# AjayGaneshC/medical-segmentation-pytorch

Hardware: AMD Instinct MI355X
Metric: images/sec (whole node) + val Dice, DUCKNet-17 352x352 at 1/2/4/8 MI355X (higher is better)
Workload: dtype bf16; 1 GPU; model=DUCKNet-17, global_batch=320, per_gpu_batch=320, seq_len=123904, step=SegTrainer.train_step, image_size=352, parallelism=dp1, impl=fused, optimizer=adam, loss=ce, syncbn=False, hipgraph=True

## Files before the change

csrc/bindings.cpp:

```cpp
#include <torch/extension.h>
#include <c10/hip/HIPStream.h>

#include <algorithm>
#include <vector>

#include "launchers.h"

namespace {

hipStream_t cur_stream() { return c10::hip::getCurrentHIPStream().stream(); }

#define CHECK_DEV(t) TORCH_CHECK((t).is_cuda() && (t).is_contiguous(), #t " must be a contiguous GPU tensor")
#define CHECK_BF16(t) CHECK_DEV(t); TORCH_CHECK((t).scalar_type() == at::kBFloat16, #t " must be bf16")
#define CHECK_F32(t) CHECK_DEV(t); TORCH_CHECK((t).scalar_type() == at::kFloat, #t " must be fp32")
#define CHECK_I64(t) CHECK_DEV(t); TORCH_CHECK((t).scalar_type() == at::kLong, #t " must be int64")

inline uint16_t* bf(const at::Tensor& t) { return reinterpret_cast<uint16_t*>(t.data_ptr()); }
inline float* f32(const at::Tensor& t) { return t.data_ptr<float>(); }
inline const float* f32_opt(const c10::optional<at::Tensor>& t) {
  if (!t.has_value() || !t->defined()) return nullptr;
  CHECK_F32(*t);
  return t->data_ptr<float>();
}
inline float* f32_opt_mut(const c10::optional<at::Tensor>& t) { return const_cast<float*>(f32_opt(t)); }

using OptTensors = std::vector<c10::optional<at::Tensor>>;

void fill_coefs(const OptTensors& cs, int n, const std::vector<int64_t>& ld, const float** out) {
  TORCH_CHECK(cs.empty() || (int)cs.size() == n, "one prologue entry per input");
  for (int i = 0; i < n; ++i) {
    out[i] = nullptr;
    if (cs.empty() || !cs[i].has_value() || !cs[i]->defined()) continue;
    CHECK_F32(*cs[i]);
    TORCH_CHECK(cs[i]->numel() >= 2 * ld[i], "prologue coefficients must hold [scale; shift] rows of the input width");
    out[i] = cs[i]->data_ptr<float>();
  }
}

bool fill_bwd(const OptTensors& ys, const OptTensors& ss, const OptTensors& ks, int n, int64_t numel, int64_t C,
// ... 1590 lines not shown
PYBIND11_MODULE(_C, m) {
  m.doc() = "MI355X (gfx950) HIP kernels for medical_segmentation_pytorch_amd";
  m.def("conv_fwd", &conv_fwd, py::arg("xs"), py::arg("wp"), py::arg("ys"), py::arg("bias"), py::arg("stat_part"),
        py::arg("dims"), py::arg("dy"), py::arg("dx"), py::arg("trans"), py::arg("xc") = OptTensors{},
        py::arg("xrelu") = 0, py::arg("accumulate") = false, py::arg("gy") = OptTensors{},
        py::arg("gs") = OptTensors{}, py::arg("gk") = OptTensors{}, py::arg("grelu") = 0);
  m.def("conv_fwd_bn", &conv_fwd_bn, py::arg("xs"), py::arg("wp"), py::arg("ys"), py::arg("stat_part"), py::arg("dims"),
        py::arg("dy"), py::arg("dx"), py::arg("bn_y"), py::arg("bn_coef"), py::arg("relu"), py::arg("gy") = OptTensors{},
        py::arg("gs") = OptTensors{}, py::arg("gk") = OptTensors{}, py::arg("grelu") = 0);
  m.def("conv_wgrad", &conv_wgrad_t, py::arg("dys"), py::arg("xs"), py::arg("dw"), py::arg("dims"), py::arg("dy"),
        py::arg("dx"), py::arg("trans"), py::arg("xc") = OptTensors{}, py::arg("xrelu") = 0,
        py::arg("gy") = OptTensors{}, py::arg("gs") = OptTensors{}, py::arg("gk") = OptTensors{}, py::arg("grelu") = 0);
  m.def("conv_wgrad_uses_halo", &conv_wgrad_uses_halo_t);
  m.def("conv_pick_mi", &conv_pick_mi);
  m.def("conv_rows_alloc", &conv_rows_alloc);
  m.def("conv_stat_blocks", &conv_stat_blocks_t, py::arg("dims"), py::arg("dy"), py::arg("dx"), py::arg("trans") = false,
        py::arg("bwd") = false, py::arg("bne") = false);
  m.def("conv_uses_halo", &conv_uses_halo_t, py::arg("dims"), py::arg("dy"), py::arg("dx"), py::arg("trans"),
        py::arg("bwd") = false);
  m.def("conv_set_halo", [](bool on) { conv_set_halo(on ? 1 : 0); });
  m.def("conv_set_halo_split", [](int64_t mode) { conv_set_halo_split((int)mode); });
  m.def("conv_set_gemm", [](bool on) { conv_gemm_set(on ? 1 : 0); });
  m.def("conv_gemm_force_cfg", [](int64_t c) { conv_gemm_force_cfg((int)c); });
  m.def("conv_gemm_num_cfgs", []() { return conv_gemm_num_cfgs(); });
  m.def("conv_gemm_stamp_buffer", [](c10::optional<at::Tensor> buf) {
    if (!buf.has_value()) return conv_gemm_stamp_buffer(nullptr, 0);
    TORCH_CHECK(buf->is_cuda() && buf->is_contiguous() && buf->scalar_type() == at::kLong && buf->dim() == 2 &&
                    buf->size(1) == 4, "conv_gemm_stamp_buffer: a contiguous int64 [blocks][4] device tensor");
    return conv_gemm_stamp_buffer(buf->data_ptr(), buf->size(0));
  });
  m.def("conv_set_wgrad_gemm", [](int64_t mode) { conv_wgrad_gemm_set((int)mode); });
  m.def("conv_wgrad_gemm_force_cfg", [](int64_t c) { conv_wgrad_gemm_force_cfg((int)c); });
  m.def("conv_wgrad_gemm_num_cfgs", []() { return conv_wgrad_gemm_num_cfgs(); });
  m.def("conv_uses_wgrad_gemm", [](std::vector<int64_t> dims, std::vector<int64_t> dy, std::vector<int64_t> dx, bool trans) {
    return conv_wgrad_gemm_ok(make_geom(dims, dy, dx), trans);
  });
  m.def("conv_uses_gemm", [](std::vector<int64_t> dims, std::vector<int64_t> dy, std::vector<int64_t> dx, bool trans) {
    return conv_gemm_ok(make_geom(dims, dy, dx), trans);
  });
  m.def("conv_set_phase", [](bool on) { conv_set_phase(on ? 1 : 0); });
  m.def("pack_weight", &pack_weight_t);
  m.def("unpack_wgrad", &unpack_wgrad_t, py::arg("src"), py::arg("dst"), py::arg("nrow"), py::arg("nch"),
        py::arg("T"), py::arg("Cpk"), py::arg("Ktot"), py::arg("t_base"), py::arg("c_base"), py::arg("s_row"),
        py::arg("s_ch"), py::arg("accumulate"), py::arg("nrep") = 1, py::arg("rep_stride") = 0);
  m.def("conv_wgrad_replicas", &conv_wgrad_replicas_t, py::arg("dims"), py::arg("dy"), py::arg("dx"), py::arg("trans"),
        py::arg("bwd") = false, py::arg("pro") = false);
  m.def("pack_batch", &pack_batch_t);
  m.def("pack_per_block", &pack_per_block);
  m.def("bn_partial_blocks", [](int64_t P, int64_t Cp) { return bn_partial_blocks(P, Cp); });
  m.def("sum_stats", &sum_stats_t, py::arg("inputs"), py::arg("out"), py::arg("part"), py::arg("P"), py::arg("Cp"),
        py::arg("coefs") = OptTensors{}, py::arg("relu_mask") = 0);
  m.def("bn_reduce_partials", &bn_reduce_partials_t);
  m.def("bn_reduce_splits", [](int64_t nblk) { return bn_reduce_splits(nblk); });
  m.def("bn_collapse", &bn_collapse_t);
  m.def("bn_finalize", &bn_finalize_t);
  m.def("bn_reduce_finalize", &bn_reduce_finalize_t);
  m.def("bn_reduce_bwd_finalize", &bn_reduce_bwd_finalize_t);
  m.def("bn_rf_chunks", [](int64_t Cp) { return bn_rf_chunks((int)Cp); });
  m.def("bn_act_apply", &bn_act_apply_t);
  m.def("bn_act_apply_relu6", &bn_act_apply_relu6_t);
  m.def("bn_add_act", &bn_add_act_t);
  m.def("gconv_fwd", &gconv_fwd_t);
  m.def("relu6", &relu6_t);
  m.def("relu6_bwd", &relu6_bwd_t);
  m.def("bn_aug_mask", &bn_aug_mask_t);
  m.def("gconv_dgrad", &gconv_dgrad_t);
// ... 155 lines not shown
```

csrc/build.py:

```python
#!/usr/bin/env python3
from __future__ import annotations

import argparse
import os
import shutil
import subprocess
import sys
import sysconfig

HERE = os.path.dirname(os.path.abspath(__file__))
ROOT = os.path.dirname(HERE)
PKG = os.path.join(ROOT, 'medical_segmentation_pytorch_amd')
VARIANT = os.environ.get('MSP_BUILD_VARIANT', '')
BUILD = os.path.join(ROOT, 'build', 'csrc' + (f'_{VARIANT}' if VARIANT else ''))
ARCH = os.environ.get('PYTORCH_ROCM_ARCH', 'gfx950').split(';')[0]
ROCM = os.environ.get('ROCM_PATH', '/opt/rocm')


def source_files():
    names = sorted(f for f in os.listdir(HERE) if f.endswith(('.hip', '.h', '.cpp')))
    return [os.path.join(HERE, f) for f in names] + [os.path.abspath(__file__)]


def sources_sha():
# ... 39 lines not shown
    tdir = os.path.dirname(torch.__file__)
    inc = [os.path.join(tdir, 'include'), os.path.join(tdir, 'include', 'torch', 'csrc', 'api', 'include')]
    return tdir, inc, int(torch._C._GLIBCXX_USE_CXX11_ABI)


def write_ninja(jobs):
    tdir, tinc, abi = torch_paths()
    pyinc = sysconfig.get_paths()['include']
    import pybind11
    hipcc = shutil.which('hipcc') or os.path.join(ROCM, 'bin', 'hipcc')
    kernels = sorted(f for f in os.listdir(HERE) if f.endswith('.hip'))
    common = f'-O3 -fPIC -std=c++17 -D_GLIBCXX_USE_CXX11_ABI={abi} -I{HERE}'
    kflags = f'{common} --offload-arch={ARCH} -munsafe-fp-atomics -Wno-unused-result'
    if VARIANT:
        kflags += ' ' + os.environ.get('MSP_BUILD_DEFINES', '')
    bflags = (f'{common} -D__HIP_PLATFORM_AMD__=1 -DUSE_ROCM=1 -DTORCH_EXTENSION_NAME=_C '
              f'-DTORCH_API_INCLUDE_EXTENSION_H -I{ROCM}/include -I{pyinc} -I{pybind11.get_include()} '
              + ' '.join(f'-isystem {p}' for p in tinc) + ' -Wno-deprecated-declarations')
    tlib = os.path.join(tdir, 'lib')
    ldflags = (f'-shared -fPIC -L{tlib} -Wl,-rpath,{tlib} -Wl,--no-as-needed -lc10 -ltorch -ltorch_cpu '
               f'-ltorch_python -lc10_hip -ltorch_hip')
    out = os.path.join(PKG, '_C.so') if not VARIANT else os.path.join(ROOT, 'build', VARIANT, '_C.so')
    os.makedirs(os.path.dirname(out), exist_ok=True)
    lines = [
        f'hipcc = {hipcc}',
        f'kflags = {kflags}',
        f'bflags = {bflags}',
        f'ldflags = {ldflags}',
        'rule hip\n  command = $hipcc $kflags -c $in -o $out\n  description = HIPCC $in',
        'rule cxx\n  command = $hipcc -x c++ $bflags -c $in -o $out\n  description = CXX $in',
        f'rule link\n  command = {shutil.which("g++") or "g++"} $in $ldflags -o $out\n  description = LINK $out',
    ]
    objs = []
    headers = ' '.join(os.path.join(HERE, h) for h in ('common.h', 'launchers.h'))
    for k in kernels:
        o = os.path.join(BUILD, k.replace('.hip', '.o'))
        lines.append(f'build {o}: hip {os.path.join(HERE, k)} | {headers}')
        objs.append(o)
    bo = os.path.join(BUILD, 'bindings.o')
    lines.append(f'build {bo}: cxx {os.path.join(HERE, "bindings.cpp")} | {headers}')
    objs.append(bo)
    so_ = os.path.join(BUILD, 'sources_sha.o')
    lines.append(f'rule cc\n  command = {shutil.which("g++") or "g++"} -O2 -fPIC -c $in -o $out\n  description = CC $in')
    lines.append(f'build {so_}: cc {os.path.join(BUILD, "sources_sha.cpp")}')
    objs.append(so_)
    lines.append(f'build {out}: link {" ".join(objs)}')
    os.makedirs(BUILD, exist_ok=True)
    path = os.path.join(BUILD, 'build.ninja')
    with open(path, 'w') as f:
        f.write('\n'.join(lines) + '\n')
    return path, out


def _mtimes(paths):
    return {p: (os.path.getmtime(p) if os.path.exists(p) else None) for p in paths}


def sha256(path):
    import hashlib
    h = hashlib.sha256()
    with open(path, 'rb') as f:
        for chunk in iter(lambda: f.read(1 << 20), b''):
            h.update(chunk)
    return h.hexdigest()


def build(jobs=None, verbose=False, force=None):
# ... 53 lines not shown
```

csrc/conv_wgrad_gemm.hip:

```cpp
#include <algorithm>

#include "common.h"
#include "launchers.h"

namespace {

typedef float f32x16_t __attribute__((ext_vector_type(16)));
typedef short s16x4_t __attribute__((ext_vector_type(4)));
typedef __attribute__((address_space(3))) uint8_t lds_u8_t;

DEVI f32x16_t mfma32(const uint4& a, const uint4& b, f32x16_t c) {
#ifdef GK_KO_MFMA
  c[0] += __uint_as_float(a.x ^ b.y);
  return c;
#else
  return __builtin_amdgcn_mfma_f32_32x32x16_bf16(as_bf16x8(a), as_bf16x8(b), c, 0, 0, 0);
#endif
}

__device__ __attribute__((aligned(64))) uint4 g_wg_zero_page[4];

DEVI void glds16(const void* src, uint32_t lds) {
#ifdef GK_KO_DMA
  return;
#endif
  unsigned keep;
  asm volatile("s_mov_b32 %0, m0\n\ts_mov_b32 m0, %2\n\ts_nop 0\n\tglobal_load_lds_dwordx4 %1, off\n\ts_mov_b32 m0, %0"
               : "=&s"(keep) : "v"(src), "s"(lds) : "memory");
}

DEVI uint2 tr_read(const uint8_t* p) {
#ifdef GK_KO_LDS
  return make_uint2((uint32_t)(uintptr_t)p, 1u);
#endif
  s16x4_t v = __builtin_amdgcn_ds_read_tr16_b64_v4i16((s16x4_t __attribute__((address_space(3)))*)(p));
  union { s16x4_t s; uint2 u; } c; c.s = v; return c.u;
}

struct FastDiv { uint32_t mul, shr; };
DEVI uint32_t fdiv_u(uint32_t n, FastDiv f) {
  return (uint32_t)(((uint64_t)__umulhi(n, f.mul) + n) >> f.shr);
}
FastDiv make_fastdiv(uint32_t d) {
  FastDiv f{0, 0};
  if (d <= 1) return f;
  uint32_t l = 0;
  while ((1ull << l) < d) ++l;
  f.mul = (uint32_t)((((1ull << l) - d) << 32) / d + 1);
  f.shr = l;
  return f;
}

constexpr int kBP = 64;

template <int R>
DEVI int chunk_swz(int row) { return R == 64 ? 0 : (R == 128 ? ((row >> 1) & 1) : (row & 3)); }

struct WgGeom {
  long M;
  int KT, n_co, n_k, stages_per_split, nstages;
  FastDiv d_ohw, d_ow;
  int kw, ty0, tys, tx0, txs;
};

template <int WM, int WN, int FM, int FN, bool PRO>
__global__ __launch_bounds__(64 * WM * WN, 2) void conv_wgrad_gemm_kernel(WgradPtrs P, float* __restrict__ dw,
                                                                          ConvGeom g, WgGeom wg) {
  constexpr int NW = WM * WN, NT = 64 * NW;
  constexpr int TCO = 32 * WM * FM, TK = 32 * WN * FN;
  constexpr int RA = TCO * 2, RB = TK * 2;
  constexpr int A_BYTES = kBP * RA, B_BYTES = kBP * RB, STAGE = A_BYTES + B_BYTES;
  constexpr int A_RPI = 1024 / RA, B_RPI = 1024 / RB;
  constexpr int A_INS = kBP / A_RPI / NW, B_INS = kBP / B_RPI / NW;
  static_assert((RA == 64 || RA == 128 || RA % 256 == 0) && (RB == 64 || RB == 128 || RB % 256 == 0), "row bytes");
  static_assert(RA <= 1024 && RB <= 1024 && A_INS * A_RPI * NW == kBP && B_INS * B_RPI * NW == kBP, "DMA split");
  static_assert(!PRO || B_RPI % 4 == 0, "prologue: one channel vector per lane (B rows <= 256 B)");
  extern __shared__ __attribute__((aligned(16))) uint8_t smem[];

  const int tid = threadIdx.x, lane = tid & 63, wave = __builtin_amdgcn_readfirstlane(tid >> 6);
  const uint32_t sbase = (uint32_t)(uintptr_t)(lds_u8_t*)smem;

  const int nwg = gridDim.x, orig = blockIdx.x;
  const int xq = nwg / 8, xr = nwg % 8, xcd = orig % 8;
  const int wgid = (xcd < xr ? xcd * (xq + 1) : xr * (xq + 1) + (xcd - xr) * xq) + orig / 8;
  const int ntile = wg.n_co * wg.n_k;
  const int split = wgid / ntile, tile = wgid - split * ntile;
  const int co_t = tile % wg.n_co, k_t = tile / wg.n_co;
  const int co0 = co_t * TCO, k0 = k_t * TK;
  const int rows = g.Go * g.Cgo, Cip = g.Gi * g.Cgi;
  const int st0 = split * wg.stages_per_split;
  const int nst = max(0, min(wg.stages_per_split, wg.nstages - st0));
  const uint16_t* zero = reinterpret_cast<const uint16_t*>(g_wg_zero_page);

  const uint16_t* a_base[A_INS];
  int a_row[A_INS];
#pragma unroll
  for (int j = 0; j < A_INS; ++j) {
    const int row = (j * NW + wave) * A_RPI + (lane * 16) / RA;
    const int slot = ((lane * 16) % RA) / 16;
    const int col = 32 * ((slot >> 2) ^ chunk_swz<RA>(row)) + 8 * (slot & 3);
    const int co = co0 + col;
    a_row[j] = row;
    if (co < rows) {
      const int og = co / g.Cgo;
      a_base[j] = P.dy[og] + (co - og * g.Cgo);
    } else {
      a_base[j] = nullptr;
    }
  }
  const uint16_t* b_base[B_INS];
  int b_row[B_INS], b_dy[B_INS], b_dx[B_INS];
  int b_ci = 0, b_gi = 0;
#pragma unroll
  for (int j = 0; j < B_INS; ++j) {
    const int row = (j * NW + wave) * B_RPI + (lane * 16) / RB;
    const int slot = ((lane * 16) % RB) / 16;
    const int col = 32 * ((slot >> 2) ^ chunk_swz<RB>(row)) + 8 * (slot & 3);
    const int k = k0 + col;
    b_row[j] = row;
    if (k < wg.KT) {
      const int t = k / Cip, rem = k - (k / Cip) * Cip;
      const int gi = rem / g.Cgi, ci = rem - gi * g.Cgi;
      const int tr = t / wg.kw, tc = t - (t / wg.kw) * wg.kw;
      b_dy[j] = wg.ty0 + tr * wg.tys;
      b_dx[j] = wg.tx0 + tc * wg.txs;
      const uint16_t* xg = P.x[0];
#pragma unroll
      for (int q = 1; q < kMaxGroups; ++q) xg = gi == q ? P.x[q] : xg;
      b_base[j] = xg + ci;
      b_ci = ci; b_gi = gi;
    } else {
      b_base[j] = nullptr; b_dy[j] = 0; b_dx[j] = 0;
    }
  }
  float psc[8], psh[8];
  bool prelu = false, pro_on = false;
  if constexpr (PRO) {
    const float* cf = P.xc[0];
#pragma unroll
    for (int q = 1; q < kMaxGroups; ++q) cf = b_gi == q ? P.xc[q] : cf;
    pro_on = cf != nullptr && b_base[0] != nullptr;
    prelu = (P.xrelu >> b_gi) & 1u;
#pragma unroll
    for (int e = 0; e < 8; ++e) { psc[e] = 1.f; psh[e] = 0.f; }
    if (pro_on) { load8f(cf + b_ci, psc); load8f(cf + g.Cgi + b_ci, psh); }
  }

  auto stage = [&](int s, uint32_t sb) -> unsigned {
    const long mb = (long)(st0 + s) * kBP;
#pragma unroll
    for (int j = 0; j < A_INS; ++j) {
      const long m = mb + a_row[j];
      const void* src = (a_base[j] != nullptr && m < wg.M) ? (const void*)(a_base[j] + m * g.Cgo) : (const void*)zero;
      glds16(src, sb + (j * NW + wave) * 1024);
    }
    unsigned ok = 0;
#pragma unroll
    for (int j = 0; j < B_INS; ++j) {
      const long m = mb + b_row[j];
      const void* src = zero;
      if (b_base[j] != nullptr && m < wg.M) {
        const uint32_t mu = (uint32_t)m;
        const uint32_t n = fdiv_u(mu, wg.d_ohw);
        const uint32_t r = mu - n * (uint32_t)(g.OH * g.OW);
        const uint32_t oh = fdiv_u(r, wg.d_ow);
        const int ow = (int)(r - oh * (uint32_t)g.OW);
        const int ih = (int)oh * g.stride + b_dy[j], iw = ow * g.stride + b_dx[j];
        if ((unsigned)ih < (unsigned)g.IH && (unsigned)iw < (unsigned)g.IW) {
          src = b_base[j] + ((long)((int)n * g.IH + ih) * g.IW + iw) * g.Cgi;
          ok |= 1u << j;
        }
      }
      glds16(src, sb + A_BYTES + (j * NW + wave) * 1024);
    }
    return ok;
  };

  const int wm = wave / WN, wn = wave - (wave / WN) * WN;
  const int gq = lane >> 4, li = lane & 15, lq = li >> 2, lp = li & 3;
  auto tr_addr = [&](int R, int row, int col) -> int {
    const int sw = R == 64 ? 0 : (R == 128 ? ((row >> 1) & 1) : (row & 3));
    return row * R + (((col >> 5) ^ sw) << 6) + ((col & 31) << 1);
  };
  int a_off[FM][2], b_off[FN][2];
#pragma unroll
  for (int i = 0; i < FM; ++i)
#pragma unroll
    for (int hh = 0; hh < 2; ++hh)
      a_off[i][hh] = tr_addr(RA, 8 * (gq >> 1) + 4 * hh + lq, wm * FM * 32 + i * 32 + 16 * (gq & 1) + 4 * lp);
#pragma unroll
  for (int j = 0; j < FN; ++j)
#pragma unroll
    for (int hh = 0; hh < 2; ++hh)
      b_off[j][hh] = A_BYTES + tr_addr(RB, 8 * (gq >> 1) + 4 * hh + lq, wn * FN * 32 + j * 32 + 16 * (gq & 1) + 4 * lp);

  f32x16_t acc[FM][FN];
#pragma unroll
  for (int i = 0; i < FM; ++i)
#pragma unroll
    for (int j = 0; j < FN; ++j)
#pragma unroll
      for (int e = 0; e < 16; ++e) acc[i][j][e] = 0.f;

  unsigned ok_cur = 0, ok_nxt = 0;
  if (nst > 0) ok_cur = stage(0, sbase);
  for (int s = 0; s < nst; ++s) {
    asm volatile("s_waitcnt vmcnt(0)" ::: "memory");
    const uint32_t cur = (s & 1) * STAGE;
    if constexpr (PRO) {
      if (pro_on) {
#pragma unroll
        for (int j = 0; j < B_INS; ++j) {
          if (!((ok_cur >> j) & 1u)) continue;
          uint4* v = reinterpret_cast<uint4*>(smem + cur + A_BYTES + (j * NW + wave) * 1024 + lane * 16);
          *v = affine8(*v, psc, psh, prelu);
        }
      }
      asm volatile("s_waitcnt lgkmcnt(0)" ::: "memory");
    }
    __builtin_amdgcn_s_barrier();
    __builtin_amdgcn_sched_barrier(0);
    if (s + 1 < nst) ok_nxt = stage(s + 1, sbase + ((s + 1) & 1) * STAGE);
    const uint8_t* sp = smem + cur;
#pragma unroll
    for (int ks = 0; ks < kBP / 16; ++ks) {
      uint4 af[FM], bf[FN];
#pragma unroll
      for (int i = 0; i < FM; ++i) {
        const uint2 lo = tr_read(sp + a_off[i][0] + ks * 16 * RA);
        const uint2 hi = tr_read(sp + a_off[i][1] + ks * 16 * RA);
        af[i] = make_uint4(lo.x, lo.y, hi.x, hi.y);
      }
#pragma unroll
      for (int j = 0; j < FN; ++j) {
        const uint2 lo = tr_read(sp + b_off[j][0] + ks * 16 * RB);
        const uint2 hi = tr_read(sp + b_off[j][1] + ks * 16 * RB);
        bf[j] = make_uint4(lo.x, lo.y, hi.x, hi.y);
      }
#pragma unroll
      for (int i = 0; i < FM; ++i)
#pragma unroll
        for (int j = 0; j < FN; ++j) acc[i][j] = mfma32(af[i], bf[j], acc[i][j]);
    }
    ok_cur = ok_nxt;
  }

  float* slab = dw + (long)split * rows * wg.KT;
  const int kc = k0 + wn * FN * 32 + (lane & 31);
  const int lh = lane >> 5;
#pragma unroll
  for (int j = 0; j < FN; ++j) {
    const int k = kc + 32 * j;
    if (k >= wg.KT) continue;
#pragma unroll
    for (int i = 0; i < FM; ++i)
#pragma unroll
      for (int e = 0; e < 16; ++e) {
        const int co = co0 + wm * FM * 32 + i * 32 + 8 * (e >> 2) + 4 * lh + (e & 3);
        if (co < rows) slab[(long)co * wg.KT + k] = acc[i][j][e];
      }
  }
}

constexpr bool wg_pro_ok(int wn, int fn) { return 32 * wn * fn <= 128; }

struct WgCfg { int wm, wn, fm, fn; };
constexpr WgCfg kWgCfgs[] = {
    {2, 2, 2, 2},
    {1, 4, 1, 1},
    {2, 2, 1, 2},
    {2, 2, 2, 1},
    {1, 4, 2, 1},
    {2, 2, 4, 1},
    {2, 4, 4, 2},
    {2, 4, 2, 2},
    {4, 2, 2, 2},
};
constexpr int kNumWgCfgs = sizeof(kWgCfgs) / sizeof(kWgCfgs[0]);

int g_wg_mode = -1;
int g_wg_cfg = -1;
constexpr long g_wg_blocks = 512;
constexpr double g_wg_stage_cost = 96.0;

void wg_env() {
  if (g_wg_mode < 0) {
    const char* e = getenv("MSP_WGRAD_GEMM");
    g_wg_mode = e == nullptr ? 1 : (e[0] == '0' ? 0 : (e[0] == '2' ? 2 : 1));
  }
}

int wg_pick(int rows, int KT, bool pro) {
  if (g_wg_cfg >= 0 && (!pro || wg_pro_ok(kWgCfgs[g_wg_cfg].wn, kWgCfgs[g_wg_cfg].fn))) return g_wg_cfg;
  int best = 0;
  double best_cost = 1e30;
  for (int c = 0; c < kNumWgCfgs; ++c) {
    if (pro && !wg_pro_ok(kWgCfgs[c].wn, kWgCfgs[c].fn)) continue;
    const int tco = 32 * kWgCfgs[c].wm * kWgCfgs[c].fm, tk = 32 * kWgCfgs[c].wn * kWgCfgs[c].fn;
    const double nt = (double)cdiv(rows, tco) * cdiv(KT, tk);
    const double cost = nt * ((double)tco * tk + g_wg_stage_cost * (tco + tk));
    if (cost < best_cost) { best_cost = cost; best = c; }
  }
  return best;
}

bool wg_tap_grid(const ConvGeom& g, WgGeom& w) {
  for (int kw = 1; kw <= g.T; ++kw) {
    if (g.T % kw != 0) continue;
    const int kh = g.T / kw;
    w.kw = kw; w.ty0 = g.dy[0]; w.tx0 = g.dx[0];
    w.tys = kh > 1 ? g.dy[kw] - g.dy[0] : 0;
    w.txs = kw > 1 ? g.dx[1] - g.dx[0] : 0;
    bool ok = true;
    for (int t = 0; t < g.T && ok; ++t) ok = g.dy[t] == w.ty0 + (t / kw) * w.tys && g.dx[t] == w.tx0 + (t % kw) * w.txs;
    if (ok) return true;
  }
  return false;
}

struct WgPlan { int cfg; WgGeom w; long blocks; int nsplit; };

WgPlan wg_plan(const ConvGeom& g, bool pro) {
  WgPlan p{};
  p.cfg = wg_pick(g.Go * g.Cgo, g.T * g.Gi * g.Cgi, pro);
  const WgCfg& c = kWgCfgs[p.cfg];
  WgGeom& w = p.w;
  (void)wg_tap_grid(g, w);
  w.M = (long)g.N * g.OH * g.OW;
  w.KT = g.T * g.Gi * g.Cgi;
  w.n_co = cdiv(g.Go * g.Cgo, 32 * c.wm * c.fm);
  w.n_k = cdiv(w.KT, 32 * c.wn * c.fn);
  w.nstages = (int)((w.M + kBP - 1) / kBP);
  const long ntile = (long)w.n_co * w.n_k;
  const long target = c.wm * c.wn >= 8 ? g_wg_blocks / 2 : g_wg_blocks;
  long ns = std::max(1L, std::min((long)w.nstages, target / std::max(1L, ntile)));
  w.stages_per_split = (int)((w.nstages + ns - 1) / ns);
  ns = (w.nstages + w.stages_per_split - 1) / w.stages_per_split;
  p.nsplit = (int)ns;
  p.blocks = ns * ntile;
  w.d_ohw = make_fastdiv((uint32_t)(g.OH * g.OW));
  w.d_ow = make_fastdiv((uint32_t)g.OW);
  return p;
}

template <int WM, int WN, int FM, int FN>
int launch_wg(const WgradPtrs& P, float* dw, const ConvGeom& g, const WgPlan& p, bool pro, hipStream_t s) {
  constexpr int LDS = 2 * kBP * (32 * WM * FM + 32 * WN * FN) * 2;
  static bool attr[2] = {false, false};
  if (pro) {
    if constexpr (!wg_pro_ok(WN, FN)) {
      return 1;
    } else {
    if (!attr[1]) {
      (void)hipFuncSetAttribute(reinterpret_cast<const void*>(&conv_wgrad_gemm_kernel<WM, WN, FM, FN, true>),
                                hipFuncAttributeMaxDynamicSharedMemorySize, LDS);
      attr[1] = true;
    }
    hipLaunchKernelGGL((conv_wgrad_gemm_kernel<WM, WN, FM, FN, true>), dim3((unsigned)p.blocks), dim3(64 * WM * WN),
                       LDS, s, P, dw, g, p.w);
    return 0;
    }
  }
  if (!attr[0]) {
    (void)hipFuncSetAttribute(reinterpret_cast<const void*>(&conv_wgrad_gemm_kernel<WM, WN, FM, FN, false>),
                              hipFuncAttributeMaxDynamicSharedMemorySize, LDS);
    attr[0] = true;
  }
  hipLaunchKernelGGL((conv_wgrad_gemm_kernel<WM, WN, FM, FN, false>), dim3((unsigned)p.blocks), dim3(64 * WM * WN), LDS,
                     s, P, dw, g, p.w);
  return 0;
}


}

bool conv_wgrad_gemm_ok(const ConvGeom& g, bool trans) {
  wg_env();
  if (!g_wg_mode || trans || g.Cgi % 8 != 0 || g.Cgo % 8 != 0) return false;
  WgGeom w{};
  if (!wg_tap_grid(g, w)) return false;
  const long M = (long)g.N * g.OH * g.OW;
  return M < (1L << 31) - 2 * kBP;
}

int conv_wgrad_gemm_replicas(const ConvGeom& g, bool pro) {
  wg_env();
  return wg_plan(g, pro).nsplit;
}

void conv_wgrad_gemm_set(int mode) { wg_env(); g_wg_mode = mode < 0 ? 0 : (mode > 2 ? 2 : mode); }
int conv_wgrad_gemm_mode() { wg_env(); return g_wg_mode; }
void conv_wgrad_gemm_force_cfg(int cfg) { wg_env(); g_wg_cfg = (cfg >= 0 && cfg < kNumWgCfgs) ? cfg : -1; }
int conv_wgrad_gemm_num_cfgs() { return kNumWgCfgs; }

int conv_wgrad_gemm(const WgradPtrs& P, float* dw, const ConvGeom& g, bool prologue, hipStream_t s) {
  const WgPlan p = wg_plan(g, prologue);
  switch (p.cfg) {
    case 0: return launch_wg<2, 2, 2, 2>(P, dw, g, p, prologue, s);
    case 1: return launch_wg<1, 4, 1, 1>(P, dw, g, p, prologue, s);
    case 2: return launch_wg<2, 2, 1, 2>(P, dw, g, p, prologue, s);
    case 3: return launch_wg<2, 2, 2, 1>(P, dw, g, p, prologue, s);
    case 4: return launch_wg<1, 4, 2, 1>(P, dw, g, p, prologue, s);
    case 5: return launch_wg<2, 2, 4, 1>(P, dw, g, p, prologue, s);
    case 6: return launch_wg<2, 4, 4, 2>(P, dw, g, p, prologue, s);
    case 7: return launch_wg<2, 4, 2, 2>(P, dw, g, p, prologue, s);
    case 8: return launch_wg<4, 2, 2, 2>(P, dw, g, p, prologue, s);
  }
  return 1;
}
```

csrc/launchers.h:

```cpp
#pragma once
#include <hip/hip_runtime.h>
#include <stdint.h>

constexpr int kMaxTaps = 49;

constexpr int kMaxGroups = 8;
struct ConvGeom {
  int N, IH, IW;
  int Gi, Cgi;
  int OH, OW;
  int Go, Cgo, Cgo_l;
  int T, Kp;
  int stride;
  int dy[kMaxTaps], dx[kMaxTaps];
};

struct ConvArgs {
  const uint16_t* x[kMaxGroups];
  uint16_t* y[kMaxGroups];
  const uint16_t* w;
  const float* bias;
  float* stat_part;
  const uint16_t* bn_y;
  const float* bn_coef;
  int bn_relu;
  const float* xc[kMaxGroups];
  unsigned xrelu;
  int accum;
  const uint16_t* gy[kMaxGroups];
  const float* gs[kMaxGroups];
  const float* gk[kMaxGroups];
  unsigned grelu;
  ConvGeom g;
};

struct WgradPtrs {
  const uint16_t* dy[kMaxGroups];
  const uint16_t* x[kMaxGroups];
  const float* xc[kMaxGroups];
  unsigned xrelu;
  const uint16_t* gy[kMaxGroups];
  const float* gs[kMaxGroups];
  const float* gk[kMaxGroups];
  unsigned grelu;
};

bool conv_wgrad_gemm_ok(const ConvGeom& g, bool trans);
int conv_wgrad_gemm_replicas(const ConvGeom& g, bool pro = false);
int conv_wgrad_gemm(const WgradPtrs& P, float* dw, const ConvGeom& g, bool prologue, hipStream_t s);
void conv_wgrad_gemm_set(int mode);
int conv_wgrad_gemm_mode();
void conv_wgrad_gemm_force_cfg(int cfg);
int conv_wgrad_gemm_num_cfgs();

int conv_pick_mi(int rows);
int conv_rows_alloc(int rows);
void conv_set_halo(int on);
void conv_set_halo_split(int mode);
void conv_set_phase(int on);
bool conv_uses_halo(const ConvGeom& g, bool trans, bool bwd = false);
long conv_stat_blocks(const ConvGeom& g, bool trans = false, bool bwd = false, bool bne = false);
bool conv_wgrad_uses_halo(const ConvGeom& g, bool trans);
int conv_igemm(const ConvArgs& a, bool trans, hipStream_t s);
const char* conv_error_string(int rc);

bool conv_gemm_ok(const ConvGeom& g, bool trans);
long conv_gemm_stat_blocks(const ConvGeom& g);
int conv_gemm(const ConvArgs& a, hipStream_t s);
int conv_gemm_phase(const ConvArgs& a, const int* tA, int KW, int s_, int py, int px, int OHf, int OWf,
                    hipStream_t s);
void conv_gemm_set(int on);
void conv_gemm_force_cfg(int cfg);
int conv_gemm_num_cfgs();
int conv_gemm_stamp_buffer(void* buf, long cap);
int conv_plan_selfcheck(int verbose);
int conv_wgrad_replicas(const ConvGeom& g, bool trans, bool bwd = false, bool pro = false);
int conv_wgrad(const uint16_t* const* dy, const uint16_t* const* x, float* dw, const ConvGeom& g, bool trans,
               const float* const* xc, unsigned xrelu, hipStream_t s, const uint16_t* const* gy = nullptr,
               const float* const* gs = nullptr, const float* const* gk = nullptr, unsigned grelu = 0);
void pack_weight(const float* src, uint16_t* dst, int nrow, int nch, int T, int Cpk, int Kp, int t_base,
                 int c_base, long s_row, long s_ch, hipStream_t s);
void pack_batch(const int64_t* jobs, const int* prefix, int njobs, int total_blocks, hipStream_t s);
int pack_per_block();
void unpack_wgrad(const float* src, float* dst, int nrow, int nch, int T, int Cpk, int Ktot, int t_base, int c_base,
                  long s_row, long s_ch, bool accumulate, int nrep, long rep_stride, hipStream_t s);

// ... 303 lines not shown
```

Measured before the change: 688.2 images/sec.

## Deepen wgrad GEMM LDS ring and replace per-stage div address math with cursor walk

The weight-gradient implicit-GEMM kernel gains configurable ring depth (NS stages) and stage size (BP), using counted vmcnt waits so several global-to-LDS loads stay in flight instead of draining to zero each stage. Per-stage fast-division address computation for the input operand is replaced by an incremental cursor that walks output positions by a fixed step, and A addresses are advanced incrementally. The two largest base configs are now mapped by default to new variants: a 4-stage ring with 32-pixel stages and a 3-stage ring with 64-pixel stages. This costs more LDS per block and adds debug/tuning bindings, with a risk of lower occupancy or added register pressure.

```diff
diff --git a/csrc/bindings.cpp b/csrc/bindings.cpp
--- a/csrc/bindings.cpp
+++ b/csrc/bindings.cpp
@@ -5,6 +5,7 @@
 #include <vector>
 
 #include "launchers.h"
+#include "wgrad_walk.h"
 
 namespace {
 
@@ -1661,6 +1662,30 @@
   m.def("conv_set_wgrad_gemm", [](int64_t mode) { conv_wgrad_gemm_set((int)mode); });
   m.def("conv_wgrad_gemm_force_cfg", [](int64_t c) { conv_wgrad_gemm_force_cfg((int)c); });
   m.def("conv_wgrad_gemm_num_cfgs", []() { return conv_wgrad_gemm_num_cfgs(); });
+  m.def("conv_wgrad_gemm_force_splits", [](int64_t n) { conv_wgrad_gemm_force_splits((int)n); });
+  m.def("conv_wgrad_gemm_set_ring", [](int64_t base, int64_t variant) { conv_wgrad_gemm_set_ring((int)base, (int)variant); });
+  m.def("conv_wgrad_gemm_cfg_info", [](int64_t cfg) {
+    int o[7];
+    conv_wgrad_gemm_cfg_info((int)cfg, o);
+    return std::vector<int64_t>(o, o + 7);
+  });
+  m.def("conv_wgrad_gemm_plan_cfg", [](std::vector<int64_t> dims, std::vector<int64_t> dy, std::vector<int64_t> dx, bool pro) {
+    return conv_wgrad_gemm_plan_cfg(make_geom(dims, dy, dx), pro);
+  });
+  m.def("wgrad_cursor_trace", [](std::vector<int64_t> dims, int64_t row, std::vector<int64_t> tap, int64_t step,
+                                 int64_t stages) {
+    TORCH_CHECK(dims.size() == 6 && tap.size() == 2 && step > 0 && row >= 0, "wgrad_cursor_trace: arguments");
+    const int N = (int)dims[0], IH = (int)dims[1], IW = (int)dims[2], OH = (int)dims[3], OW = (int)dims[4];
+    const WgWalk w = wg_walk_make(N, IH, IW, OH, OW, (int)dims[5], (int)step);
+    WgCursor c = wg_cursor_init(w, (int)(row / (OH * OW)), (int)((row % (OH * OW)) / OW), (int)(row % OW));
+    std::vector<std::pair<bool, int64_t>> out;
+    for (int64_t s = 0; s < stages; ++s) {
+      const bool in = wg_cursor_in(w, c, (int)tap[0], (int)tap[1]);
+      out.emplace_back(in, in ? (int64_t)(uint32_t)(c.base + (uint32_t)((int)tap[0] * IW + (int)tap[1])) : (int64_t)-1);
+      wg_cursor_advance(w, c);
+    }
+    return out;
+  });
   m.def("conv_uses_wgrad_gemm", [](std::vector<int64_t> dims, std::vector<int64_t> dy, std::vector<int64_t> dx, bool trans) {
     return conv_wgrad_gemm_ok(make_geom(dims, dy, dx), trans);
   });
diff --git a/csrc/build.py b/csrc/build.py
--- a/csrc/build.py
+++ b/csrc/build.py
@@ -95,7 +95,7 @@
         f'rule link\n  command = {shutil.which("g++") or "g++"} $in $ldflags -o $out\n  description = LINK $out',
     ]
     objs = []
-    headers = ' '.join(os.path.join(HERE, h) for h in ('common.h', 'launchers.h'))
+    headers = ' '.join(os.path.join(HERE, h) for h in ('common.h', 'launchers.h', 'wgrad_walk.h'))
     for k in kernels:
         o = os.path.join(BUILD, k.replace('.hip', '.o'))
         lines.append(f'build {o}: hip {os.path.join(HERE, k)} | {headers}')
diff --git a/csrc/conv_wgrad_gemm.hip b/csrc/conv_wgrad_gemm.hip
--- a/csrc/conv_wgrad_gemm.hip
+++ b/csrc/conv_wgrad_gemm.hip
@@ -2,6 +2,7 @@
 
 #include "common.h"
 #include "launchers.h"
+#include "wgrad_walk.h"
 
 namespace {
 
@@ -51,7 +52,7 @@
   return f;
 }
 
-constexpr int kBP = 64;
+constexpr int kSplitPx = 64;
 
 template <int R>
 DEVI int chunk_swz(int row) { return R == 64 ? 0 : (R == 128 ? ((row >> 1) & 1) : (row & 3)); }
@@ -61,20 +62,27 @@
   int KT, n_co, n_k, stages_per_split, nstages;
   FastDiv d_ohw, d_ow;
   int kw, ty0, tys, tx0, txs;
+  WgWalk walk;
 };
 
-template <int WM, int WN, int FM, int FN, bool PRO>
+template <int WM, int WN, int FM, int FN, bool PRO, int NS, int BP>
 __global__ __launch_bounds__(64 * WM * WN, 2) void conv_wgrad_gemm_kernel(WgradPtrs P, float* __restrict__ dw,
                                                                           ConvGeom g, WgGeom wg) {
   constexpr int NW = WM * WN, NT = 64 * NW;
   constexpr int TCO = 32 * WM * FM, TK = 32 * WN * FN;
   constexpr int RA = TCO * 2, RB = TK * 2;
-  constexpr int A_BYTES = kBP * RA, B_BYTES = kBP * RB, STAGE = A_BYTES + B_BYTES;
+  constexpr int A_BYTES = BP * RA, B_BYTES = BP * RB, STAGE = A_BYTES + B_BYTES;
   constexpr int A_RPI = 1024 / RA, B_RPI = 1024 / RB;
-  constexpr int A_INS = kBP / A_RPI / NW, B_INS = kBP / B_RPI / NW;
+  constexpr int A_STEP = A_RPI * NW, B_STEP = B_RPI * NW;
+  constexpr int A_INS = BP / A_STEP, B_INS = BP / B_STEP, INS = A_INS + B_INS;
+  static_assert(NS >= 2 && (BP == 32 || BP == 64) && kSplitPx % BP == 0, "ring shape");
   static_assert((RA == 64 || RA == 128 || RA % 256 == 0) && (RB == 64 || RB == 128 || RB % 256 == 0), "row bytes");
-  static_assert(RA <= 1024 && RB <= 1024 && A_INS * A_RPI * NW == kBP && B_INS * B_RPI * NW == kBP, "DMA split");
+  static_assert(RA <= 1024 && RB <= 1024 && A_INS >= 1 && B_INS >= 1 && A_INS * A_STEP == BP && B_INS * B_STEP == BP,
+                "DMA split");
+  static_assert(A_STEP % 4 == 0 && B_STEP % 4 == 0, "one channel column per lane");
   static_assert(!PRO || B_RPI % 4 == 0, "prologue: one channel vector per lane (B rows <= 256 B)");
+  static_assert(NS <= 4 && (NS - 2) * INS < 64, "counted vmcnt (the wait ladder below goes to 2 * INS)");
+  static_assert(!PRO || (NS - 1) * B_INS <= 32, "prologue: in-image bits of the stages in flight");
   extern __shared__ __attribute__((aligned(16))) uint8_t smem[];
 
   const int tid = threadIdx.x, lane = tid & 63, wave = __builtin_amdgcn_readfirstlane(tid >> 6);
@@ -89,91 +97,100 @@
   const int co0 = co_t * TCO, k0 = k_t * TK;
   const int rows = g.Go * g.Cgo, Cip = g.Gi * g.Cgi;
   const int st0 = split * wg.stages_per_split;
-  const int nst = max(0, min(wg.stages_per_split, wg.nstages - st0));
-  const uint16_t* zero = reinterpret_cast<const uint16_t*>(g_wg_zero_page);
-
-  const uint16_t* a_base[A_INS];
-  int a_row[A_INS];
-#pragma unroll
-  for (int j = 0; j < A_INS; ++j) {
-    const int row = (j * NW + wave) * A_RPI + (lane * 16) / RA;
+  const int nst = max(0, min(wg.stages_per_split, wg.nstages - st0)) * (kSplitPx / BP);
+  const uint32_t m0 = (uint32_t)st0 * kSplitPx;
+  const char* zero = reinterpret_cast<const char*>(g_wg_zero_page);
+  asm volatile("" : "+s"(zero));
+
+  const char* a_ptr = zero;
+  int a_rem = 0;
+  {
+    const int row = wave * A_RPI + (lane * 16) / RA;
     const int slot = ((lane * 16) % RA) / 16;
-    const int col = 32 * ((slot >> 2) ^ chunk_swz<RA>(row)) + 8 * (slot & 3);
-    const int co = co0 + col;
-    a_row[j] = row;
+    const int co = co0 + 32 * ((slot >> 2) ^ chunk_swz<RA>(row)) + 8 * (slot & 3);
     if (co < rows) {
       const int og = co / g.Cgo;
-      a_base[j] = P.dy[og] + (co - og * g.Cgo);
-    } else {
-      a_base[j] = nullptr;
-    }
-  }
-  const uint16_t* b_base[B_INS];
-  int b_row[B_INS], b_dy[B_INS], b_dx[B_INS];
-  int b_ci = 0, b_gi = 0;
-#pragma unroll
-  for (int j = 0; j < B_INS; ++j) {
-    const int row = (j * NW + wave) * B_RPI + (lane * 16) / RB;
+      const long m = (long)m0 + row;
+      a_ptr = reinterpret_cast<const char*>(P.dy[og] + (co - og * g.Cgo) + m * g.Cgo);
+      a_rem = (int)(wg.M - m);
+    }
+  }
+  const char* b_ptr = zero;
+  int b_dy = 0, b_dx = 0, b_ci = 0, b_gi = 0;
+  bool b_on = false;
+  WgCursor cur{wg.walk.N, 0, 0, 0u};
+  {
+    const int row = wave * B_RPI + (lane * 16) / RB;
     const int slot = ((lane * 16) % RB) / 16;
-    const int col = 32 * ((slot >> 2) ^ chunk_swz<RB>(row)) + 8 * (slot & 3);
-    const int k = k0 + col;
-    b_row[j] = row;
+    const int k = k0 + 32 * ((slot >> 2) ^ chunk_swz<RB>(row)) + 8 * (slot & 3);
     if (k < wg.KT) {
       const int t = k / Cip, rem = k - (k / Cip) * Cip;
       const int gi = rem / g.Cgi, ci = rem - gi * g.Cgi;
       const int tr = t / wg.kw, tc = t - (t / wg.kw) * wg.kw;
-      b_dy[j] = wg.ty0 + tr * wg.tys;
-      b_dx[j] = wg.tx0 + tc * wg.txs;
+      b_dy = wg.ty0 + tr * wg.tys;
+      b_dx = wg.tx0 + tc * wg.txs;
       const uint16_t* xg = P.x[0];
 #pragma unroll
       for (int q = 1; q < kMaxGroups; ++q) xg = gi == q ? P.x[q] : xg;
-      b_base[j] = xg + ci;
-      b_ci = ci; b_gi = gi;
-    } else {
-      b_base[j] = nullptr; b_dy[j] = 0; b_dx[j] = 0;
-    }
-  }
+      b_ptr = reinterpret_cast<const char*>(xg + ci + ((long)b_dy * g.IW + b_dx) * g.Cgi);
+      b_ci = ci; b_gi = gi; b_on = true;
+      const uint32_t mu = m0 + (uint32_t)row;
+      const uint32_t n = fdiv_u(mu, wg.d_ohw);
+      const uint32_t r = mu - n * (uint32_t)(g.OH * g.OW);
+      const uint32_t oh = fdiv_u(r, wg.d_ow);
+      cur = wg_cursor_init(wg.walk, (int)n, (int)oh, (int)(r - oh * (uint32_t)g.OW));
+    }
+  }
+  const uint32_t cgi2 = (uint32_t)g.Cgi * 2u;
   float psc[8], psh[8];
   bool prelu = false, pro_on = false;
   if constexpr (PRO) {
     const float* cf = P.xc[0];
 #pragma unroll
     for (int q = 1; q < kMaxGroups; ++q) cf = b_gi == q ? P.xc[q] : cf;
-    pro_on = cf != nullptr && b_base[0] != nullptr;
+    pro_on = cf != nullptr && b_on;
     prelu = (P.xrelu >> b_gi) & 1u;
 #pragma unroll
     for (int e = 0; e < 8; ++e) { psc[e] = 1.f; psh[e] = 0.f; }
     if (pro_on) { load8f(cf + b_ci, psc); load8f(cf + g.Cgi + b_ci, psh); }
-  }
-
-  auto stage = [&](int s, uint32_t sb) -> unsigned {
-    const long mb = (long)(st0 + s) * kBP;
-#pragma unroll
-    for (int j = 0; j < A_INS; ++j) {
-      const long m = mb + a_row[j];
-      const void* src = (a_base[j] != nullptr && m < wg.M) ? (const void*)(a_base[j] + m * g.Cgo) : (const void*)zero;
-      glds16(src, sb + (j * NW + wave) * 1024);
-    }
-    unsigned ok = 0;
+#pragma unroll
+    for (int e = 0; e < 8; ++e) asm volatile("" : "+v"(psc[e]), "+v"(psh[e]));
+  }
+
+  int a_m = 0;
+  uint64_t a_off = 0;
+  const uint64_t a_ins_b = (uint64_t)A_STEP * g.Cgo * 2u;
+  const char* src_a[A_INS];
+  const char* src_b[B_INS];
+  unsigned ok_p = 0;
+  auto prep = [&]() {
+#pragma unroll
+    for (int j = 0; j < A_INS; ++j) src_a[j] = (a_m + j * A_STEP < a_rem) ? a_ptr + (a_off + j * a_ins_b) : zero;
+    a_m += BP;
+    a_off += A_INS * a_ins_b;
+    ok_p = 0;
 #pragma unroll
     for (int j = 0; j < B_INS; ++j) {
-      const long m = mb + b_row[j];
-      const void* src = zero;
-      if (b_base[j] != nullptr && m < wg.M) {
-        const uint32_t mu = (uint32_t)m;
-        const uint32_t n = fdiv_u(mu, wg.d_ohw);
-        const uint32_t r = mu - n * (uint32_t)(g.OH * g.OW);
-        const uint32_t oh = fdiv_u(r, wg.d_ow);
-        const int ow = (int)(r - oh * (uint32_t)g.OW);
-        const int ih = (int)oh * g.stride + b_dy[j], iw = ow * g.stride + b_dx[j];
-        if ((unsigned)ih < (unsigned)g.IH && (unsigned)iw < (unsigned)g.IW) {
-          src = b_base[j] + ((long)((int)n * g.IH + ih) * g.IW + iw) * g.Cgi;
-          ok |= 1u << j;
-        }
-      }
-      glds16(src, sb + A_BYTES + (j * NW + wave) * 1024);
-    }
-    return ok;
+      const bool in = wg_cursor_in(wg.walk, cur, b_dy, b_dx);
+      uint64_t p = (uint64_t)(uintptr_t)b_ptr + (uint64_t)cur.base * cgi2;
+      asm("" : "+v"(p));
+      src_b[j] = in ? reinterpret_cast<const char*>(p) : zero;
+      ok_p |= (in ? 1u : 0u) << j;
+      wg_cursor_advance(wg.walk, cur);
+    }
+#ifdef GK_KO_ADDR
+#pragma unroll
+    for (int j = 0; j < A_INS; ++j) src_a[j] = zero;
+#pragma unroll
+    for (int j = 0; j < B_INS; ++j) src_b[j] = zero;
+#endif
+  };
+  auto issue = [&](uint32_t sb) -> unsigned {
+#pragma unroll
+    for (int j = 0; j < A_INS; ++j) glds16(src_a[j], sb + (j * NW + wave) * 1024);
+#pragma unroll
+    for (int j = 0; j < B_INS; ++j) glds16(src_b[j], sb + A_BYTES + (j * NW + wave) * 1024);
+    return ok_p;
   };
 
   const int wm = wave / WN, wn = wave - (wave / WN) * WN;
@@ -182,17 +199,17 @@
     const int sw = R == 64 ? 0 : (R == 128 ? ((row >> 1) & 1) : (row & 3));
     return row * R + (((col >> 5) ^ sw) << 6) + ((col & 31) << 1);
   };
-  int a_off[FM][2], b_off[FN][2];
+  int a_off_l[FM][2], b_off_l[FN][2];
 #pragma unroll
   for (int i = 0; i < FM; ++i)
 #pragma unroll
     for (int hh = 0; hh < 2; ++hh)
-      a_off[i][hh] = tr_addr(RA, 8 * (gq >> 1) + 4 * hh + lq, wm * FM * 32 + i * 32 + 16 * (gq & 1) + 4 * lp);
+      a_off_l[i][hh] = tr_addr(RA, 8 * (gq >> 1) + 4 * hh + lq, wm * FM * 32 + i * 32 + 16 * (gq & 1) + 4 * lp);
 #pragma unroll
   for (int j = 0; j < FN; ++j)
 #pragma unroll
     for (int hh = 0; hh < 2; ++hh)
-      b_off[j][hh] = A_BYTES + tr_addr(RB, 8 * (gq >> 1) + 4 * hh + lq, wn * FN * 32 + j * 32 + 16 * (gq & 1) + 4 * lp);
+      b_off_l[j][hh] = A_BYTES + tr_addr(RB, 8 * (gq >> 1) + 4 * hh + lq, wn * FN * 32 + j * 32 + 16 * (gq & 1) + 4 * lp);
 
   f32x16_t acc[FM][FN];
 #pragma unroll
@@ -202,17 +219,27 @@
 #pragma unroll
       for (int e = 0; e < 16; ++e) acc[i][j][e] = 0.f;
 
-  unsigned ok_cur = 0, ok_nxt = 0;
-  if (nst > 0) ok_cur = stage(0, sbase);
+  unsigned okq = 0;
+#pragma unroll
+  for (int p = 0; p < NS - 1; ++p)
+    if (p < nst) {
+      prep();
+      okq |= issue(sbase + p * STAGE) << (PRO ? p * B_INS : 0);
+    }
+  prep();
+  int cur_i = 0, iss_i = NS - 1;
   for (int s = 0; s < nst; ++s) {
-    asm volatile("s_waitcnt vmcnt(0)" ::: "memory");
-    const uint32_t cur = (s & 1) * STAGE;
+    const int ahead = min(nst - 1 - s, NS - 2);
+    if (NS >= 4 && ahead >= 2) asm volatile("s_waitcnt vmcnt(%0)" ::"n"(NS >= 4 ? 2 * INS : 0) : "memory");
+    else if (NS >= 3 && ahead >= 1) asm volatile("s_waitcnt vmcnt(%0)" ::"n"(NS >= 3 ? INS : 0) : "memory");
+    else asm volatile("s_waitcnt vmcnt(0)" ::: "memory");
+    const uint32_t cur_b = (uint32_t)cur_i * STAGE;
     if constexpr (PRO) {
       if (pro_on) {
 #pragma unroll
         for (int j = 0; j < B_INS; ++j) {
-          if (!((ok_cur >> j) & 1u)) continue;
-          uint4* v = reinterpret_cast<uint4*>(smem + cur + A_BYTES + (j * NW + wave) * 1024 + lane * 16);
+          if (!((okq >> j) & 1u)) continue;
+          uint4* v = reinterpret_cast<uint4*>(smem + cur_b + A_BYTES + (j * NW + wave) * 1024 + lane * 16);
           *v = affine8(*v, psc, psh, prelu);
         }
       }
@@ -220,21 +247,24 @@
     }
     __builtin_amdgcn_s_barrier();
     __builtin_amdgcn_sched_barrier(0);
-    if (s + 1 < nst) ok_nxt = stage(s + 1, sbase + ((s + 1) & 1) * STAGE);
-    const uint8_t* sp = smem + cur;
-#pragma unroll
-    for (int ks = 0; ks < kBP / 16; ++ks) {
+    unsigned okn = 0;
+    if (s + NS - 1 < nst) okn = issue(sbase + (uint32_t)iss_i * STAGE);
+    if constexpr (PRO) okq = (okq >> B_INS) | (okn << ((NS - 2) * B_INS));
+    prep();
+    const uint8_t* sp = smem + cur_b;
+#pragma unroll
+    for (int ks = 0; ks < BP / 16; ++ks) {
       uint4 af[FM], bf[FN];
 #pragma unroll
       for (int i = 0; i < FM; ++i) {
-        const uint2 lo = tr_read(sp + a_off[i][0] + ks * 16 * RA);
-        const uint2 hi = tr_read(sp + a_off[i][1] + ks * 16 * RA);
+        const uint2 lo = tr_read(sp + a_off_l[i][0] + ks * 16 * RA);
+        const uint2 hi = tr_read(sp + a_off_l[i][1] + ks * 16 * RA);
         af[i] = make_uint4(lo.x, lo.y, hi.x, hi.y);
       }
 #pragma unroll
       for (int j = 0; j < FN; ++j) {
-        const uint2 lo = tr_read(sp + b_off[j][0] + ks * 16 * RB);
-        const uint2 hi = tr_read(sp + b_off[j][1] + ks * 16 * RB);
+        const uint2 lo = tr_read(sp + b_off_l[j][0] + ks * 16 * RB);
+        const uint2 hi = tr_read(sp + b_off_l[j][1] + ks * 16 * RB);
         bf[j] = make_uint4(lo.x, lo.y, hi.x, hi.y);
       }
 #pragma unroll
@@ -242,7 +272,8 @@
 #pragma unroll
         for (int j = 0; j < FN; ++j) acc[i][j] = mfma32(af[i], bf[j], acc[i][j]);
     }
-    ok_cur = ok_nxt;
+    cur_i = cur_i + 1 == NS ? 0 : cur_i + 1;
+    iss_i = iss_i + 1 == NS ? 0 : iss_i + 1;
   }
 
   float* slab = dw + (long)split * rows * wg.KT;
@@ -264,22 +295,28 @@
 
 constexpr bool wg_pro_ok(int wn, int fn) { return 32 * wn * fn <= 128; }
 
-struct WgCfg { int wm, wn, fm, fn; };
+struct WgCfg { int wm, wn, fm, fn, ns, bp, base; };
 constexpr WgCfg kWgCfgs[] = {
-    {2, 2, 2, 2},
-    {1, 4, 1, 1},
-    {2, 2, 1, 2},
-    {2, 2, 2, 1},
-    {1, 4, 2, 1},
-    {2, 2, 4, 1},
-    {2, 4, 4, 2},
-    {2, 4, 2, 2},
-    {4, 2, 2, 2},
+    {2, 2, 2, 2, 2, 64, 0},
+    {1, 4, 1, 1, 2, 64, 1},
+    {2, 2, 1, 2, 2, 64, 2},
+    {2, 2, 2, 1, 2, 64, 3},
+    {1, 4, 2, 1, 2, 64, 4},
+    {2, 2, 4, 1, 2, 64, 5},
+    {2, 4, 4, 2, 2, 64, 6},
+    {2, 4, 2, 2, 2, 64, 7},
+    {4, 2, 2, 2, 2, 64, 8},
+    {2, 4, 4, 2, 4, 32, 6},
+    {4, 2, 2, 2, 3, 64, 8},
 };
 constexpr int kNumWgCfgs = sizeof(kWgCfgs) / sizeof(kWgCfgs[0]);
+constexpr int kNumWgBase = 9;
+constexpr int kWgRingDefault[kNumWgBase] = {0, 1, 2, 3, 4, 5, 9, 7, 10};
+int g_wg_ring[kNumWgBase] = {0, 1, 2, 3, 4, 5, 9, 7, 10};
 
 int g_wg_mode = -1;
 int g_wg_cfg = -1;
+int g_wg_splits = -1;
 constexpr long g_wg_blocks = 512;
 constexpr double g_wg_stage_cost = 96.0;
 
@@ -294,14 +331,14 @@
   if (g_wg_cfg >= 0 && (!pro || wg_pro_ok(kWgCfgs[g_wg_cfg].wn, kWgCfgs[g_wg_cfg].fn))) return g_wg_cfg;
   int best = 0;
   double best_cost = 1e30;
-  for (int c = 0; c < kNumWgCfgs; ++c) {
+  for (int c = 0; c < kNumWgBase; ++c) {
     if (pro && !wg_pro_ok(kWgCfgs[c].wn, kWgCfgs[c].fn)) continue;
     const int tco = 32 * kWgCfgs[c].wm * kWgCfgs[c].fm, tk = 32 * kWgCfgs[c].wn * kWgCfgs[c].fn;
     const double nt = (double)cdiv(rows, tco) * cdiv(KT, tk);
     const double cost = nt * ((double)tco * tk + g_wg_stage_cost * (tco + tk));
     if (cost < best_cost) { best_cost = cost; best = c; }
   }
-  return best;
+  return g_wg_ring[best];
 }
 
 bool wg_tap_grid(const ConvGeom& g, WgGeom& w) {
@@ -330,47 +367,50 @@
   w.KT = g.T * g.Gi * g.Cgi;
   w.n_co = cdiv(g.Go * g.Cgo, 32 * c.wm * c.fm);
   w.n_k = cdiv(w.KT, 32 * c.wn * c.fn);
-  w.nstages = (int)((w.M + kBP - 1) / kBP);
+  w.nstages = (int)((w.M + kSplitPx - 1) / kSplitPx);
   const long ntile = (long)w.n_co * w.n_k;
   const long target = c.wm * c.wn >= 8 ? g_wg_blocks / 2 : g_wg_blocks;
   long ns = std::max(1L, std::min((long)w.nstages, target / std::max(1L, ntile)));
+  if (g_wg_splits > 0) ns = std::min((long)w.nstages, (long)g_wg_splits);
   w.stages_per_split = (int)((w.nstages + ns - 1) / ns);
   ns = (w.nstages + w.stages_per_split - 1) / w.stages_per_split;
   p.nsplit = (int)ns;
   p.blocks = ns * ntile;
   w.d_ohw = make_fastdiv((uint32_t)(g.OH * g.OW));
   w.d_ow = make_fastdiv((uint32_t)g.OW);
+  const int b_step = (1024 / (64 * c.wn * c.fn)) * c.wm * c.wn;
+  w.walk = wg_walk_make(g.N, g.IH, g.IW, g.OH, g.OW, g.stride, b_step);
   return p;
 }
 
-template <int WM, int WN, int FM, int FN>
+template <int WM, int WN, int FM, int FN, int NS, int BP>
 int launch_wg(const WgradPtrs& P, float* dw, const ConvGeom& g, const WgPlan& p, bool pro, hipStream_t s) {
-  constexpr int LDS = 2 * kBP * (32 * WM * FM + 32 * WN * FN) * 2;
+  constexpr int LDS = NS * BP * (32 * WM * FM + 32 * WN * FN) * 2;
+  static_assert(LDS <= 160 * 1024, "LDS per block");
   static bool attr[2] = {false, false};
   if (pro) {
     if constexpr (!wg_pro_ok(WN, FN)) {
       return 1;
     } else {
     if (!attr[1]) {
-      (void)hipFuncSetAttribute(reinterpret_cast<const void*>(&conv_wgrad_gemm_kernel<WM, WN, FM, FN, true>),
+      (void)hipFuncSetAttribute(reinterpret_cast<const void*>(&conv_wgrad_gemm_kernel<WM, WN, FM, FN, true, NS, BP>),
                                 hipFuncAttributeMaxDynamicSharedMemorySize, LDS);
       attr[1] = true;
     }
-    hipLaunchKernelGGL((conv_wgrad_gemm_kernel<WM, WN, FM, FN, true>), dim3((unsigned)p.blocks), dim3(64 * WM * WN),
-                       LDS, s, P, dw, g, p.w);
+    hipLaunchKernelGGL((conv_wgrad_gemm_kernel<WM, WN, FM, FN, true, NS, BP>), dim3((unsigned)p.blocks),
+                       dim3(64 * WM * WN), LDS, s, P, dw, g, p.w);
     return 0;
     }
   }
   if (!attr[0]) {
-    (void)hipFuncSetAttribute(reinterpret_cast<const void*>(&conv_wgrad_gemm_kernel<WM, WN, FM, FN, false>),
+    (void)hipFuncSetAttribute(reinterpret_cast<const void*>(&conv_wgrad_gemm_kernel<WM, WN, FM, FN, false, NS, BP>),
                               hipFuncAttributeMaxDynamicSharedMemorySize, LDS);
     attr[0] = true;
   }
-  hipLaunchKernelGGL((conv_wgrad_gemm_kernel<WM, WN, FM, FN, false>), dim3((unsigned)p.blocks), dim3(64 * WM * WN), LDS,
-                     s, P, dw, g, p.w);
+  hipLaunchKernelGGL((conv_wgrad_gemm_kernel<WM, WN, FM, FN, false, NS, BP>), dim3((unsigned)p.blocks),
+                     dim3(64 * WM * WN), LDS, s, P, dw, g, p.w);
   return 0;
 }
-
 
 }
 
@@ -380,7 +420,7 @@
   WgGeom w{};
   if (!wg_tap_grid(g, w)) return false;
   const long M = (long)g.N * g.OH * g.OW;
-  return M < (1L << 31) - 2 * kBP;
+  return M < (1L << 31) - 2 * kSplitPx && (long)g.N * g.IH * g.IW < (1L << 31);
 }
 
 int conv_wgrad_gemm_replicas(const ConvGeom& g, bool pro) {
@@ -392,19 +432,33 @@
 int conv_wgrad_gemm_mode() { wg_env(); return g_wg_mode; }
 void conv_wgrad_gemm_force_cfg(int cfg) { wg_env(); g_wg_cfg = (cfg >= 0 && cfg < kNumWgCfgs) ? cfg : -1; }
 int conv_wgrad_gemm_num_cfgs() { return kNumWgCfgs; }
+void conv_wgrad_gemm_force_splits(int n) { wg_env(); g_wg_splits = n > 0 ? n : -1; }
+void conv_wgrad_gemm_set_ring(int base, int variant) {
+  wg_env();
+  if (base < 0 || base >= kNumWgBase) return;
+  const bool ok = variant >= 0 && variant < kNumWgCfgs && kWgCfgs[variant].base == base;
+  g_wg_ring[base] = ok ? variant : kWgRingDefault[base];
+}
+void conv_wgrad_gemm_cfg_info(int cfg, int out[7]) {
+  const WgCfg& c = kWgCfgs[cfg >= 0 && cfg < kNumWgCfgs ? cfg : 0];
+  out[0] = c.wm; out[1] = c.wn; out[2] = c.fm; out[3] = c.fn; out[4] = c.ns; out[5] = c.bp; out[6] = c.base;
+}
+int conv_wgrad_gemm_plan_cfg(const ConvGeom& g, bool pro) { wg_env(); return wg_plan(g, pro).cfg; }
 
 int conv_wgrad_gemm(const WgradPtrs& P, float* dw, const ConvGeom& g, bool prologue, hipStream_t s) {
   const WgPlan p = wg_plan(g, prologue);
   switch (p.cfg) {
-    case 0: return launch_wg<2, 2, 2, 2>(P, dw, g, p, prologue, s);
-    case 1: return launch_wg<1, 4, 1, 1>(P, dw, g, p, prologue, s);
-    case 2: return launch_wg<2, 2, 1, 2>(P, dw, g, p, prologue, s);
-    case 3: return launch_wg<2, 2, 2, 1>(P, dw, g, p, prologue, s);
-    case 4: return launch_wg<1, 4, 2, 1>(P, dw, g, p, prologue, s);
-    case 5: return launch_wg<2, 2, 4, 1>(P, dw, g, p, prologue, s);
-    case 6: return launch_wg<2, 4, 4, 2>(P, dw, g, p, prologue, s);
-    case 7: return launch_wg<2, 4, 2, 2>(P, dw, g, p, prologue, s);
-    case 8: return launch_wg<4, 2, 2, 2>(P, dw, g, p, prologue, s);
+    case 0: return launch_wg<2, 2, 2, 2, 2, 64>(P, dw, g, p, prologue, s);
+    case 1: return launch_wg<1, 4, 1, 1, 2, 64>(P, dw, g, p, prologue, s);
+    case 2: return launch_wg<2, 2, 1, 2, 2, 64>(P, dw, g, p, prologue, s);
+    case 3: return launch_wg<2, 2, 2, 1, 2, 64>(P, dw, g, p, prologue, s);
+    case 4: return launch_wg<1, 4, 2, 1, 2, 64>(P, dw, g, p, prologue, s);
+    case 5: return launch_wg<2, 2, 4, 1, 2, 64>(P, dw, g, p, prologue, s);
+    case 6: return launch_wg<2, 4, 4, 2, 2, 64>(P, dw, g, p, prologue, s);
+    case 7: return launch_wg<2, 4, 2, 2, 2, 64>(P, dw, g, p, prologue, s);
+    case 8: return launch_wg<4, 2, 2, 2, 2, 64>(P, dw, g, p, prologue, s);
+    case 9: return launch_wg<2, 4, 4, 2, 4, 32>(P, dw, g, p, prologue, s);
+    case 10: return launch_wg<4, 2, 2, 2, 3, 64>(P, dw, g, p, prologue, s);
   }
   return 1;
 }
diff --git a/csrc/launchers.h b/csrc/launchers.h
--- a/csrc/launchers.h
+++ b/csrc/launchers.h
@@ -52,6 +52,10 @@
 int conv_wgrad_gemm_mode();
 void conv_wgrad_gemm_force_cfg(int cfg);
 int conv_wgrad_gemm_num_cfgs();
+void conv_wgrad_gemm_force_splits(int n);
+void conv_wgrad_gemm_set_ring(int base, int variant);
+void conv_wgrad_gemm_cfg_info(int cfg, int out[7]);
+int conv_wgrad_gemm_plan_cfg(const ConvGeom& g, bool pro);
 
 int conv_pick_mi(int rows);
 int conv_rows_alloc(int rows);
diff --git a/csrc/wgrad_walk.h b/csrc/wgrad_walk.h
--- /dev/null
+++ b/csrc/wgrad_walk.h
@@ -0,0 +1,48 @@
+#pragma once
+#include <hip/hip_runtime.h>
+#include <stdint.h>
+
+struct WgWalk {
+  int N, IH, IW;
+  int ows_lim, ohs_lim;
+  int stride;
+  int dows, dohs, dn;
+  uint32_t dbase;
+  uint32_t wrap_w;
+  uint32_t wrap_h;
+};
+struct WgCursor { int n, ohs, ows; uint32_t base; };
+
+__host__ __device__ inline WgWalk wg_walk_make(int N, int IH, int IW, int OH, int OW, int stride, int step) {
+  WgWalk w;
+  w.N = N; w.IH = IH; w.IW = IW; w.stride = stride;
+  w.ows_lim = OW * stride; w.ohs_lim = OH * stride;
+  w.dows = (step % OW) * stride;
+  w.dohs = ((step / OW) % OH) * stride;
+  w.dn = step / (OH * OW);
+  w.dbase = (uint32_t)w.dows + (uint32_t)w.dohs * (uint32_t)IW + (uint32_t)w.dn * (uint32_t)(IH * IW);
+  w.wrap_w = (uint32_t)(stride * IW) - (uint32_t)(OW * stride);
+  w.wrap_h = (uint32_t)(IH * IW) - (uint32_t)(OH * stride) * (uint32_t)IW;
+  return w;
+}
+__host__ __device__ inline WgCursor wg_cursor_init(const WgWalk& w, int n, int oh, int ow) {
+  WgCursor c;
+  c.n = n; c.ohs = oh * w.stride; c.ows = ow * w.stride;
+  c.base = ((uint32_t)n * (uint32_t)w.IH + (uint32_t)c.ohs) * (uint32_t)w.IW + (uint32_t)c.ows;
+  return c;
+}
+__host__ __device__ inline void wg_cursor_advance(const WgWalk& w, WgCursor& c) {
+  c.ows += w.dows;
+  c.base += w.dbase;
+  const bool cw = c.ows >= w.ows_lim;
+  c.ows -= cw ? w.ows_lim : 0;
+  c.ohs += w.dohs + (cw ? w.stride : 0);
+  c.base += cw ? w.wrap_w : 0u;
+  const bool ch = c.ohs >= w.ohs_lim;
+  c.ohs -= ch ? w.ohs_lim : 0;
+  c.n += w.dn + (ch ? 1 : 0);
+  c.base += ch ? w.wrap_h : 0u;
+}
+__host__ __device__ inline bool wg_cursor_in(const WgWalk& w, const WgCursor& c, int dy, int dx) {
+  return (int)(c.n < w.N) & (int)((unsigned)(c.ohs + dy) < (unsigned)w.IH) & (int)((unsigned)(c.ows + dx) < (unsigned)w.IW);
+}
```

Measured after the change: 696.9 images/sec, median of 6. 1.3% higher.
